# openshift/kubernetes-autoscaler

Hardware: NVIDIA H100
Metric: pod x node predicate evals/sec (higher is better)
Workload: dtype int64

## Files before the change

### kubernetes-autoscaler_b200/csrc/engine.h

```cpp
#pragma once
#include <cuda_runtime.h>

#include <climits>
#include <cstdint>
#include <string>
#include <vector>

#include "../../include/caengine.h"
#include "dyn.cuh"
#include "tables.cuh"

namespace cae {

constexpr int FEAS_MAX_W = 4;
constexpr int FEAS_LUT_MAX_ROWS = 1024;
constexpr int FEAS_TW = 16;

void set_error(const std::string& msg);

struct alignas(16) GroupRec {
  int32_t n, spec, sc, dc;
  uint32_t flags;
  int32_t pad[2];
  int32_t kcap;
  unsigned long long pconf, pbit;
  int64_t req[CAE_MAX_RES];
  float rinv[CAE_MAX_RES];
};
static_assert(sizeof(GroupRec) == 144, "GroupRec is fetched as nine 16-byte chunks");
enum : uint32_t { GREC_HAS_PORTS = 1u, GREC_FEEDS = 2u, GREC_HOST_SPREAD = 4u };

struct GroupRecSrc {
  int has_dyn, n_act;
  int act_dim[CAE_MAX_RES];
  const int32_t *spec_sc, *spec_dc, *pc_of;
  const unsigned long long* port_conf;
};
__device__ __forceinline__ GroupRec build_group_rec(const DevObjects& o, const GroupRecSrc& s, int spec, int n, bool feeds) {
  GroupRec r{};
  r.n = n;
  r.kcap = INT_MAX;
  if (n <= 0) return r;
  r.spec = spec;
  r.sc = s.spec_sc[spec];
  r.dc = s.has_dyn ? s.spec_dc[spec] : 0;
  const int plist = o.ps_port_list[spec];
  const bool has_ports = o.port_off[plist + 1] > o.port_off[plist];
  r.pconf = has_ports ? s.port_conf[plist] : 0ull;
  r.pbit = has_ports ? (1ull << s.pc_of[plist]) : 0ull;
  r.flags = (has_ports ? GREC_HAS_PORTS : 0u) | (feeds ? GREC_FEEDS : 0u) | (o.ps_hostname_spread[spec] ? GREC_HOST_SPREAD : 0u);
  for (int a = 0; a < s.n_act; ++a) {
    r.req[a] = o.ps_req[(size_t)spec * R + s.act_dim[a]];
    r.rinv[a] = r.req[a] > 0 ? __frcp_rn(__ll2float_rn(r.req[a])) : 0.f;
    if (r.req[a] >> 32) r.kcap = min(r.kcap, (int)(LLONG_MAX / r.req[a]));
  }
  return r;
}
constexpr int ORDER_NOT_ON_FRESH = 1 << 30;

#define CAE_CUDA(expr)                                                                        \
  do {                                                                                        \
    cudaError_t _e = (expr);                                                                  \
    if (_e != cudaSuccess) {                                                                  \
      cae::set_error(std::string(#expr) + ": " + cudaGetErrorString(_e));                     \
      return -1;                                                                              \
    }                                                                                         \
  } while (0)

#define CAE_KERNEL_OK()                                                                       \
  do {                                                                                        \
    cudaError_t _e = cudaGetLastError();                                                      \
    if (_e != cudaSuccess) {                                                                  \
      cae::set_error(std::string(__func__) + ": " + cudaGetErrorString(_e));                  \
      return -1;                                                                              \
    }                                                                                         \
  } while (0)

struct Arena {
  struct Chunk { void* dev = nullptr; void* host = nullptr; size_t size = 0, used = 0, flushed = 0; };
  std::vector<Chunk> chunks;
  size_t cur = 0;
  size_t min_chunk = (size_t)32 << 20;
  bool mirrored = false;
  int alloc(void** dev, void** stage, size_t bytes);
  int flush(cudaStream_t st, int64_t* bytes);
  void reset();
  void release();
};

struct Engine {
  cae_config cfg{};
  cudaStream_t stream = nullptr;
  cudaEvent_t ev0 = nullptr, ev1 = nullptr, ev2 = nullptr, ev3 = nullptr;
  Arena up;
  Arena pup;
  Arena scratch;
  Engine() { up.mirrored = true; pup.mirrored = true; }
  DynTables dyn;
  const uint8_t* d_spec_used = nullptr;
  const int32_t* d_dc_ngroups = nullptr;
  int64_t* d_c_free = nullptr;
  int32_t* d_c_slots = nullptr;
  cae_stats stats{};
  bool loaded = false;

  int N = 0, T = 0, E = 0, P = 0, U = 0;
  int A = 0;
  int act_dim[CAE_MAX_RES] = {0};
  int SC = 0, DC = 0;
  int Tw = 0;
  int Twp = 0;
  int p_begin = 0, p_end = 0;
  int t_begin = 0, t_end = 0;
  int Pl = 0, Plw = 0;
  bool has_dynamic = false;

  DevObjects dobj{};
  StaticClass* d_sclass = nullptr;
  uint8_t* d_pre_code = nullptr;
  uint32_t* d_pre_ok = nullptr;
  int32_t* d_spec_sc = nullptr;
  int32_t* d_spec_dc = nullptr;
  uint8_t* d_post_code = nullptr;
  uint32_t* d_post_ok = nullptr;
  int W = 0;
  uint32_t* d_spec_w = nullptr;
  uint32_t* d_pod_w = nullptr;
  uint16_t* d_pod_row = nullptr;
  int feas_B = 0;
  uint32_t feas_fstart = 0;
  uint8_t feas_sword[32] = {0}, feas_sshift[32] = {0};
  uint32_t* d_tslice = nullptr;
  int lut_rows = 0;
  int lut_base[CAE_MAX_RES] = {0};
  uint8_t lut_word[CAE_MAX_RES] = {0}, lut_shift[CAE_MAX_RES] = {0};
  uint32_t lut_mask[CAE_MAX_RES] = {0};
  uint32_t* d_rlut = nullptr;
  long long* d_tmpl_cost = nullptr;
  int32_t* d_perm = nullptr;
  bool force_bitslice = false;
  int32_t* d_pod_sc = nullptr;
  int32_t* d_pod_dc = nullptr;
  int64_t* d_tmpl_free = nullptr;
  int64_t* d_tmpl_free_all = nullptr;
  int32_t* d_tmpl_slots = nullptr;
  uint32_t* d_fit_bits = nullptr;
  uint8_t* d_reasons = nullptr;
  int32_t* d_fit_count = nullptr;
  int32_t* d_fit_acc = nullptr;
  int32_t* d_chunk_done = nullptr;
  uint8_t* d_group_reason = nullptr;
  bool group_reason_valid = false;
  int32_t* d_counts2 = nullptr;
  int32_t* d_sched = nullptr;
  int32_t* d_order = nullptr;
  int32_t* d_order_n = nullptr;
  GroupRec* d_grec = nullptr;
  double* d_waste = nullptr;
  int32_t* d_max_nodes = nullptr;
  int32_t* d_last_index_buf = nullptr;
  const int32_t* d_last_index_in = nullptr;
  int32_t* d_last_index_out = nullptr;
  int32_t* d_pc_of = nullptr;
  unsigned long long* d_port_conf = nullptr;
  int pack_cap = 1 << 30;
  struct DevBuf {
    void* p = nullptr;
    size_t cap = 0;
    DevBuf() = default;
    DevBuf(const DevBuf&) = delete;
    DevBuf& operator=(const DevBuf&) = delete;
    ~DevBuf() { if (p) cudaFree(p); }
  };
  struct PinnedBuf {
    void* p = nullptr;
    size_t cap = 0;
    cudaEvent_t ev = nullptr;
    PinnedBuf() = default;
    PinnedBuf(const PinnedBuf&) = delete;
    PinnedBuf& operator=(const PinnedBuf&) = delete;
    ~PinnedBuf() { if (p) cudaFreeHost(p); if (ev) cudaEventDestroy(ev); }
  };
  struct Slab { DevBuf buf; size_t sig = 0, zeroed = 0; };
  Slab pack_slab, fm_slab;
  DevBuf fm_blob;
  DevBuf rm_state;
  PinnedBuf rm_stage;
  std::vector<int32_t> rm_owner, rm_seen;
  DevBuf x_rows;
  DevBuf x_price;
  static constexpr int PEER_MAX = 8, PEER_CAP = 1 << 16;
  int32_t* d_xbuf = nullptr;
  int peer_world = 0;
  int32_t* peer_base[PEER_MAX] = {nullptr};
  int64_t peer_step = 0;
  int32_t* d_work_counter = nullptr;
  const int32_t *h_group_off = nullptr, *h_pend_spec = nullptr;
  std::vector<int32_t> h_group_spec;
  bool groups_homogeneous = true;
  std::vector<uint8_t> h_spec_pending;
  int cap_P = 0, cap_E = 0, cap_Pl = 0;
  PinnedBuf pending_stage;
  std::vector<int64_t> h_spec_req;
  int num_podspecs = 0;
  struct NodeHost {
    int32_t num_values = 0, num_labelsets = 0, num_taint_lists = 0, taint_entries = 0;
    std::vector<int32_t> ls_off, ls_key, ls_val;
    std::vector<int32_t> pod_cnt;
    int64_t pod_total = 0;
    std::vector<uint8_t> spec_used;
    std::vector<uint8_t> spec_anti;
    std::vector<int32_t> key_val;
    std::vector<int32_t> tkey_val;
    std::vector<int32_t> q_k;
    std::vector<int32_t> dom_scratch;
    std::vector<int32_t> tmpl_ls;
  } nh;
  struct PodHost {
    int32_t hostname_key = -1, num_res = 0;
    int32_t num_namespaces = 0, num_reqs = 0, req_vals = 0, num_selectors = 0, num_naff = 0, num_naff_terms = 0, fields = 0;
    int32_t num_tol_lists = 0, tol_entries = 0, num_aterms = 0, aterm_ns = 0;
    std::vector<int32_t> ps_namespace, ps_labelset, ps_tol_list, ps_naff, ps_node_name, ps_port_list, ps_pts_list, ps_aff_list,
        ps_anti_list;
    std::vector<int32_t> port_off, pts_off, pts_key, aff_off, aterm_key;
  } ph;
  DevBuf pd_tab[49];
  PinnedBuf pd_stage;
  DevBuf pd_blob;
  DevBuf pd_used;
  DevBuf nd_tab[9];
  DevBuf nd_off[2], nd_spec[2];
  DevBuf nd_cnt, nd_didx, nd_cub, nd_blob;
  PinnedBuf nd_stage;
  DevBuf ch_nodes[2];
  DevBuf ch_pre;
  DevBuf ch_dyn;
  DevBuf sim_dev;
  PinnedBuf sim_stage;
  int sm_count = 132;
  int smem_optin = 227 * 1024;
  size_t hbm_bytes = (size_t)80 << 30;
};

int devbuf_reserve(Engine* e, Engine::DevBuf& b, size_t bytes);
int pinned_reserve(Engine* e, Engine::PinnedBuf& b, size_t bytes);

int launch_class_matrix(Engine* e);
int launch_class_matrix_cols(Engine* e, const int32_t* d_cols, int ncols);
int launch_dynamic_recount(Engine* e, const int32_t* d_cols, int ncols);
struct NodeDeltaDev {
  int nd, na;
  const int32_t *row, *name;
  const int32_t *labelset, *taint_list, *allowed, *cslots, *pod_off, *pod_spec;
  const uint8_t* unsched;
  const int64_t *alloc, *cfree;
};
int launch_node_rows(Engine* e, const NodeDeltaDev& d, int64_t total);
int launch_node_churn(Engine* e, const NodeDeltaDev& d, const int32_t* src, int N_new, int64_t total);
int launch_pre_ok_bits(Engine* e);
int launch_post_bits(Engine* e);
int launch_dynamic_tables(Engine* e, const uint8_t* d_spec_used, const int32_t* d_dc_ngroups);
int launch_expand_pods(Engine* e);
int launch_port_conflicts(Engine* e, int num_port_lists);
int launch_feasibility(Engine* e, bool want_reasons);
int launch_group_feasibility(Engine* e);
int launch_order(Engine* e);
int launch_group_records(Engine* e);
GroupRecSrc group_rec_src(const Engine* e);
int launch_binpack(Engine* e);
struct FilterLaunch {
  int runs, n_pods, last_index, break_on_failure, nctrl;
  const int32_t *run_off, *pods, *hint, *cls, *class_ctrl;
  const uint8_t* node_ok;
  int32_t *assigned, *out, *ctrl_cnt;
  uint8_t *class_mark, *ctrl_over;
};
int launch_filter(Engine* e, const FilterLaunch& f);
struct RemovalLaunch {
  int ncand, persist, ncls, nctrl, log_cap, last_index, n_move;
  const int32_t *cand, *move_off, *move_pod, *hint, *cls, *class_ctrl;
  const uint8_t* dest_ok;
  int32_t *result, *log, *out;
};
struct RemovalState {
  int ncand, persist, log_cap, li_in, ncls, nctrl;
  const int32_t *cand, *move_off, *move_pod;
  const uint8_t* dest_ok;
  int32_t *result, *log, *out;
  int64_t* cfree;
  int32_t* cslots;
  unsigned long long* cports;
  uint8_t *live, *live_w;
  int32_t* rank;
  int32_t *ccnt, *cpres, *ctot;
  int32_t *wcnt, *wpres, *wtot;
  int32_t* stat;
  int32_t* hint;
  int32_t *head, *tail, *next;
  int32_t* run_off;
  GroupRecSrc grs;
};
int launch_removals(Engine* e, const RemovalLaunch& r);
struct RankArgs {
  int A, N, T, Tw, Twp, W, lut_rows, feas_B, Bpad;
  int act[CAE_MAX_RES], f_word[CAE_MAX_RES], f_shift[CAE_MAX_RES], f_bits[CAE_MAX_RES], lut_base[CAE_MAX_RES];
  uint32_t lut_mask[CAE_MAX_RES];
  int rv_off[CAE_MAX_RES + 1];
  uint8_t sword[32], sshift[32];
};
int launch_rank_tables(Engine* e, const RankArgs& a, const int64_t* d_rvals, uint32_t* d_tmpl_w);
int pd_resident_specs(Engine* e, int S, uint8_t* h_used, int32_t* h_labelset);
int launch_price(Engine* e, const cae_price_inputs& in_dev, const int32_t* d_node_count, const int32_t* d_sched, const int32_t* d_order,
                 double* d_score);
int launch_waste(Engine* e, const int32_t* d_node_count, const int32_t* d_sched, double* d_waste);
constexpr int SIM_KMAX = 2 * CAE_MAX_RES + 3;
struct SimLaunch {
  double ratio[3];
  const int32_t *res_sig, *lab_sig, *free_dims;
  int32_t* flags;
  const int64_t* cap;
  int32_t* status;
  unsigned long long* sum;
  int32_t* count;
  uint32_t* bits;
  double* x;
  uint32_t* sched;
};
int launch_similar(Engine* e, const SimLaunch& s);

}
```

### kubernetes-autoscaler_b200/csrc/feas.cu

```cuda
#include <algorithm>
#include <climits>

#include "engine.h"

namespace cae {

struct LutLayout {
  int A, rows;
  int base[CAE_MAX_RES];
  uint32_t mask[CAE_MAX_RES];
  uint8_t word[CAE_MAX_RES], shift[CAE_MAX_RES];
};

static LutLayout lut_layout(const Engine* e) {
  LutLayout lay{};
  lay.A = e->A;
  lay.rows = e->lut_rows;
  for (int d = 0; d < e->A; ++d) {
    lay.base[d] = e->lut_base[d]; lay.mask[d] = e->lut_mask[d]; lay.word[d] = e->lut_word[d]; lay.shift[d] = e->lut_shift[d];
  }
  return lay;
}

__global__ void expand_pods_kernel(const int32_t* __restrict__ pend_spec, int p_begin, int Pl, int W, LutLayout lay,
                                   const uint32_t* __restrict__ spec_w, const int32_t* __restrict__ spec_sc,
                                   const int32_t* __restrict__ spec_dc, uint32_t* __restrict__ pod_w,
                                   uint16_t* __restrict__ pod_row, int32_t* __restrict__ pod_sc, int32_t* __restrict__ pod_dc) {
  int p = blockIdx.x * blockDim.x + threadIdx.x;
  if (p >= Pl) return;
  int spec = pend_spec[p_begin + p];
  for (int w = 0; w < W; ++w) pod_w[(size_t)w * Pl + p] = spec_w[(size_t)spec * FEAS_MAX_W + w];
  for (int d = 0; d < lay.A; ++d) {
    const int row = lay.base[d] + (int)((spec_w[(size_t)spec * FEAS_MAX_W + lay.word[d]] >> lay.shift[d]) & lay.mask[d]);
    pod_row[(size_t)d * Pl + p] = (uint16_t)min(row, 0xFFFF);
  }
  pod_sc[p] = spec_sc[spec];
  pod_dc[p] = spec_dc[spec];
}

int launch_expand_pods(Engine* e) {
  if (e->Pl == 0) return 0;
  expand_pods_kernel<<<(e->Pl + 255) / 256, 256, 0, e->stream>>>(e->dobj.pend_spec, e->p_begin, e->Pl, e->W, lut_layout(e), e->d_spec_w,
                                                                   e->d_spec_sc, e->d_spec_dc, e->d_pod_w, e->d_pod_row, e->d_pod_sc, e->d_pod_dc);
  e->stats.kernel_launches++;
  CAE_KERNEL_OK();
  return 0;
}

constexpr int K1_TW = FEAS_TW;
constexpr int K1_TCHUNK = K1_TW * 32;
constexpr int K1_LPITCH = K1_TW + 1;

struct PeerPush {
  int world, rank;
  int tag;
  int2* data[8];
  const int2* self;
  int32_t* done_ctr;
  int32_t* status;
};

struct K1Args {
  int Pl, Plw, T, Tw, Twp, N, U, W;
  int G, gq, gr;
  const uint32_t* pod_w;
  const uint16_t* pod_row;
  const int32_t *pod_sc, *pod_dc;
  const uint32_t *tslice, *rlut;
  const int32_t* tmpl_slots;
  const uint32_t *pre_ok, *post_ok;
  const uint8_t *pre_code, *post_code;
  uint32_t* fit_bits;
  int32_t *fit_count, *fit_acc, *chunk_done;
  uint8_t* reasons;
};

__device__ __forceinline__ int k1_ld_acquire_sys(const int32_t* p) {
  int v;
  asm volatile("ld.acquire.sys.global.s32 %0, [%1];" : "=r"(v) : "l"(p) : "memory");
  return v;
}
__device__ __forceinline__ void k1_red_release_sys(int32_t* p, int v) {
  asm volatile("red.release.sys.global.add.s32 [%0], %1;" ::"l"(p), "r"(v) : "memory");
}
__device__ __forceinline__ void k1_st_volatile_v2(int2* p, int x, int y) {
  asm volatile("st.volatile.global.v2.s32 [%0], {%1, %2};" ::"l"(p), "r"(x), "r"(y) : "memory");
}
__device__ __forceinline__ int2 k1_ld_volatile_v2(const int2* p) {
  int2 v;
  asm volatile("ld.volatile.global.v2.s32 {%0, %1}, [%2];" : "=r"(v.x), "=r"(v.y) : "l"(p) : "memory");
  return v;
}
__device__ __forceinline__ unsigned long long k1_globaltimer() {
  unsigned long long t;
  asm volatile("mov.u64 %0, %%globaltimer;" : "=l"(t));
  return t;
}

#ifdef CAE_K1_PROF
constexpr int K1_PROF_MAX_BLOCKS = 8192, K1_PROF_STAMPS = 5;
__device__ unsigned long long k1_prof[1 + K1_PROF_STAMPS * K1_PROF_MAX_BLOCKS];
#define K1_STAMP(i)                                                                                 \
  do {                                                                                              \
    const int b_ = blockIdx.y * gridDim.x + blockIdx.x;                                             \
    if (threadIdx.x == 0 && b_ < K1_PROF_MAX_BLOCKS) k1_prof[1 + K1_PROF_STAMPS * b_ + (i)] = k1_globaltimer(); \
  } while (0)
__global__ void k1_prof_mark_kernel() { k1_prof[0] = k1_globaltimer(); }
#else
#define K1_STAMP(i) do {} while (0)
#endif

__device__ __forceinline__ void k1_finish(const K1Args& a, const PeerPush& pp, const int32_t* s_cnt, int t0, int tid, int nthreads) {
  __shared__ int s_flag;
  for (int i = tid; i < K1_TCHUNK; i += nthreads) {
    const int c = s_cnt[i];
    if (c && t0 + i < a.T) atomicAdd(&a.fit_acc[t0 + i], c);
  }
  __syncthreads();
  if (tid == 0) {
    __threadfence();
    s_flag = atomicAdd(&a.chunk_done[blockIdx.y], 1) == (int)gridDim.x - 1;
  }
  __syncthreads();
  if (!s_flag) return;
  __threadfence();
  for (int i = tid; i < K1_TCHUNK; i += nthreads) {
    const int t = t0 + i;
    if (t < a.T) {
      a.fit_count[t] = __ldcg(&a.fit_acc[t]);
      a.fit_acc[t] = 0;
    }
  }
  if (tid == 0) a.chunk_done[blockIdx.y] = 0;
  if (!pp.world) return;
  __syncthreads();
  if (tid == 0) {
    __threadfence();
    s_flag = atomicAdd(pp.done_ctr, 1) == (int)gridDim.y - 1;
  }
  __syncthreads();
  if (!s_flag) return;
  __threadfence();
  const int tag = pp.tag;
#pragma unroll
  for (int r = 0; r < Engine::PEER_MAX; ++r) {
    if (r < pp.world) {
      int2* dst = pp.data[r] + (size_t)pp.rank * Engine::PEER_CAP;
      for (int t = tid; t < a.T; t += nthreads) k1_st_volatile_v2(dst + t, __ldcg(&a.fit_count[t]), tag);
    }
  }
  const int2* mine = pp.self;
  const unsigned long long t0ns = k1_globaltimer();
  int ok = 1;
  for (int t = tid; t < a.T && ok; t += nthreads) {
    int2 x[Engine::PEER_MAX];
    unsigned pending = 0;
#pragma unroll
    for (int r = 0; r < Engine::PEER_MAX; ++r)
      if (r < pp.world) x[r] = k1_ld_volatile_v2(mine + (size_t)r * Engine::PEER_CAP + t);
#pragma unroll
    for (int r = 0; r < Engine::PEER_MAX; ++r)
      if (r < pp.world && x[r].y != tag) pending |= 1u << r;
    for (int spins = 0; pending; ) {
#pragma unroll
      for (int r = 0; r < Engine::PEER_MAX; ++r)
        if ((pending >> r) & 1u) {
          x[r] = k1_ld_volatile_v2(mine + (size_t)r * Engine::PEER_CAP + t);
          if (x[r].y == tag) pending &= ~(1u << r);
        }
      if (pending && (++spins & 1023) == 0 && k1_globaltimer() - t0ns > 2000000000ull) { ok = 0; break; }
    }
    int v = 0;
#pragma unroll
    for (int r = 0; r < Engine::PEER_MAX; ++r)
      if (r < pp.world) v += x[r].x;
    if (ok) a.fit_count[t] = v;
  }
  if (!ok) atomicExch(pp.status, 1);
  if (tid == 0) *pp.done_ctr = 0;
}

struct TransposeConsts { uint32_t sel16, sel8, amt[3], keep[3]; };

__device__ __forceinline__ uint32_t opaque(uint32_t v) {
  uint32_t r;
  asm volatile("mov.b32 %0, %1;" : "=r"(r) : "r"(v));
  return r;
}

__device__ __forceinline__ TransposeConsts transpose_consts(int lane) {
  TransposeConsts c;
  c.sel16 = opaque((lane & 16) ? 0x3276u : 0x5410u);
  c.sel8 = opaque((lane & 8) ? 0x3715u : 0x6240u);
#pragma unroll
  for (int i = 0; i < 3; ++i) {
    const int s = 4 >> i;
    const uint32_t lowmask = s == 4 ? 0x0F0F0F0Fu : s == 2 ? 0x33333333u : 0x55555555u;
    c.amt[i] = opaque((lane & s) ? (uint32_t)s : (uint32_t)(32 - s));
    c.keep[i] = opaque((lane & s) ? ~lowmask : lowmask);
  }
  return c;
}

__device__ __forceinline__ uint32_t bitselect(uint32_t x, uint32_t y, uint32_t keep) {
  uint32_t r;
  asm("lop3.b32 %0, %1, %2, %3, 0xE4;" : "=r"(r) : "r"(x), "r"(y), "r"(keep));
  return r;
}

__device__ __forceinline__ void warp_transpose32x2(uint32_t& a, uint32_t& b, const TransposeConsts& c) {
  uint32_t ya = __shfl_xor_sync(0xffffffffu, a, 16), yb = __shfl_xor_sync(0xffffffffu, b, 16);
  a = __byte_perm(a, ya, c.sel16);
  b = __byte_perm(b, yb, c.sel16);
  ya = __shfl_xor_sync(0xffffffffu, a, 8);
  yb = __shfl_xor_sync(0xffffffffu, b, 8);
  a = __byte_perm(a, ya, c.sel8);
  b = __byte_perm(b, yb, c.sel8);
#pragma unroll
  for (int i = 0; i < 3; ++i) {
    ya = __shfl_xor_sync(0xffffffffu, __funnelshift_l(a, a, c.amt[i]), 4 >> i);
    yb = __shfl_xor_sync(0xffffffffu, __funnelshift_l(b, b, c.amt[i]), 4 >> i);
    a = bitselect(a, ya, c.keep[i]);
    b = bitselect(b, yb, c.keep[i]);
  }
}

__device__ __forceinline__ uint32_t warp_transpose32(uint32_t x, int lane) {
#pragma unroll
  for (int s = 16; s >= 1; s >>= 1) {
    const uint32_t lowmask = s == 16 ? 0x0000FFFFu : s == 8 ? 0x00FF00FFu : s == 4 ? 0x0F0F0F0Fu : s == 2 ? 0x33333333u : 0x55555555u;
    const uint32_t y = __shfl_xor_sync(0xffffffffu, x, s);
    x = (lane & s) ? ((x & ~lowmask) | ((y & ~lowmask) >> s)) : ((x & lowmask) | ((y & lowmask) << s));
  }
  return x;
}

template <int A, bool REASONS>
constexpr int k1_lut_warps_per_sm() { return REASONS ? 16 : (A == 0 || A > 5) ? 32 : 48; }

template <int A, bool REASONS, int NW>
__global__ void __launch_bounds__(NW * 32, k1_lut_warps_per_sm<A, REASONS>() / NW)
feasibility_lut_kernel(K1Args a, int rows, PeerPush pp) {
  extern __shared__ uint32_t k1_smem[];
  constexpr int NT = NW * 32;
  constexpr int PAD = K1_TCHUNK + 32 / NW;
  uint32_t* s_lut = k1_smem;
  uint32_t* s_out = s_lut + (size_t)max(rows, 1) * K1_LPITCH;
  int32_t* s_cnt = reinterpret_cast<int32_t*>(s_out + NW * PAD);
  const int tid = threadIdx.x, lane = tid & 31, warp = tid >> 5;
  const int tw0 = blockIdx.y * K1_TW;
  const int t0 = tw0 * 32;
  const int pwb = (int)blockIdx.x * a.gq + min((int)blockIdx.x, a.gr);
  const int npw = a.gq + ((int)blockIdx.x < a.gr ? 1 : 0);
  const int p = (pwb + warp) * 32 + lane;
  const bool valid = warp < npw && p < a.Pl;
  K1_STAMP(0);

#pragma unroll 1
  for (int i = tid; i < rows * K1_TW; i += NT) {
    const int row = i / K1_TW, w = i % K1_TW;
    s_lut[row * K1_LPITCH + w] = a.rlut[(size_t)row * a.Twp + tw0 + w];
  }
  for (int i = tid; i < K1_TCHUNK; i += NT) s_cnt[i] = 0;

  int off[A > 0 ? A : 1];
#pragma unroll
  for (int d = 0; d < A; ++d) off[d] = valid ? (int)a.pod_row[(size_t)d * a.Pl + p] * K1_LPITCH : 0;
  const int sc = valid ? a.pod_sc[p] : 0;
  const int dc = valid ? a.pod_dc[p] : 0;
  uint32_t cls[K1_TW];
  {
    const uint4* pre = reinterpret_cast<const uint4*>(a.pre_ok + (size_t)sc * a.Twp + tw0);
    const uint4* post = reinterpret_cast<const uint4*>(a.post_ok + (size_t)dc * a.Twp + tw0);
#pragma unroll
    for (int q = 0; q < K1_TW / 4; ++q) {
      uint4 u = make_uint4(0, 0, 0, 0);
      if (valid) {
        const uint4 x = __ldg(pre + q), y = __ldg(post + q);
        u = make_uint4(x.x & y.x, x.y & y.y, x.z & y.z, x.w & y.w);
      }
      cls[4 * q + 0] = u.x; cls[4 * q + 1] = u.y; cls[4 * q + 2] = u.z; cls[4 * q + 3] = u.w;
    }
  }
  const TransposeConsts tc = transpose_consts(lane);
  __syncthreads();
  K1_STAMP(1);

#pragma unroll
  for (int tw = 0; tw < K1_TW; tw += 2) {
    uint32_t fit0 = 0xffffffffu, fit1 = 0xffffffffu;
#pragma unroll
    for (int d = 0; d < A; ++d) {
      fit0 &= s_lut[off[d] + tw];
      fit1 &= s_lut[off[d] + tw + 1];
    }
    if (REASONS) {
#pragma unroll
      for (int h = 0; h < 2; ++h) {
        const int wglob = tw0 + tw + h;
        const uint32_t fit = h ? fit1 : fit0;
        if (valid && wglob < a.Tw) {
          for (int j = 0; j < 32; ++j) {
            const int t = wglob * 32 + j;
            if (t >= a.T) break;
            uint8_t rs = a.pre_code[(size_t)sc * a.U + a.N + t] & 0x0F;
            if (rs == 0) rs = (!((fit >> j) & 1u) || a.tmpl_slots[t] < 1) ? CAE_R_FIT : a.post_code[(size_t)dc * a.T + t];
            a.reasons[(size_t)t * a.Pl + p] = rs;
          }
        }
      }
    }
    uint32_t c0 = fit0 & cls[tw], c1 = fit1 & cls[tw + 1];
    warp_transpose32x2(c0, c1, tc);
    s_out[warp * PAD + tw * 32 + lane] = c0;
    s_out[warp * PAD + (tw + 1) * 32 + lane] = c1;
    atomicAdd(&s_cnt[tw * 32 + lane], __popc(c0));
    atomicAdd(&s_cnt[(tw + 1) * 32 + lane], __popc(c1));
  }
  __syncthreads();
  K1_STAMP(2);
  if (a.fit_bits) {
    const int wv = tid % NW;
    if (wv < npw) {
      uint32_t* dst = a.fit_bits + (size_t)(t0 + tid / NW) * a.Plw + pwb + wv;
      const uint32_t* src = s_out + wv * PAD + tid / NW;
      const size_t stride = (size_t)32 * a.Plw;
      const int kmax = min(K1_TCHUNK / 32, (a.T - t0 - tid / NW + 31) / 32);
#pragma unroll 4
      for (int k = 0; k < kmax; ++k, dst += stride, src += 32) *dst = *src;
    }
  }
  K1_STAMP(3);
  k1_finish(a, pp, s_cnt, t0, tid, NT);
  K1_STAMP(4);
}

constexpr int K1_THREADS = 256;
constexpr int K1_WARPS = K1_THREADS / 32;
constexpr int K1_PAD = K1_TCHUNK + 4;

struct FeasLayout {
  uint32_t fstart;
  int nb;
  uint8_t sword[32], sshift[32];
};

template <int B, bool REASONS>
__global__ void __launch_bounds__(K1_THREADS)
feasibility_kernel(K1Args a, FeasLayout lay, PeerPush pp) {
  __shared__ uint32_t s_sl[B > 0 ? B : 1][K1_TW];
  __shared__ uint32_t s_out[K1_WARPS][K1_PAD];
  __shared__ int32_t s_cnt[K1_TCHUNK];
  const int tid = threadIdx.x, lane = tid & 31, warp = tid >> 5;
  const int p = blockIdx.x * K1_THREADS + tid;
  const int tw0 = blockIdx.y * K1_TW;
  const int t0 = tw0 * 32;

  for (int i = tid; i < B * K1_TW; i += K1_THREADS) {
    const int b = i / K1_TW, w = i % K1_TW;
    s_sl[b][w] = (tw0 + w < a.Tw) ? a.tslice[(size_t)b * a.Tw + tw0 + w] : 0u;
  }
  for (int i = tid; i < K1_TCHUNK; i += K1_THREADS) s_cnt[i] = 0;
  const bool valid = p < a.Pl;
  uint32_t r[B > 0 ? B : 1];
  {
    uint32_t pw[FEAS_MAX_W];
#pragma unroll
    for (int w = 0; w < FEAS_MAX_W; ++w) pw[w] = (valid && w < a.W) ? a.pod_w[(size_t)w * a.Pl + p] : 0u;
#pragma unroll
    for (int b = 0; b < B; ++b) {
      const uint32_t word = lay.sword[b] == 0 ? pw[0] : lay.sword[b] == 1 ? pw[1] : lay.sword[b] == 2 ? pw[2] : pw[3];
      r[b] = b < lay.nb ? 0u - ((word >> lay.sshift[b]) & 1u) : 0u;
    }
  }
  const int sc = valid ? a.pod_sc[p] : 0;
  const int dc = valid ? a.pod_dc[p] : 0;
  __syncthreads();

#pragma unroll 1
  for (int tw = 0; tw < K1_TW; ++tw) {
    const int wglob = tw0 + tw;
    uint32_t row = 0;
    if (wglob < a.Tw) {
      uint32_t gt = 0, eq = 0;
#pragma unroll
      for (int b = 0; b < B; ++b) {
        const uint32_t f = s_sl[b][tw];
        if ((lay.fstart >> b) & 1u) eq = 0xffffffffu;
        gt |= eq & r[b] & ~f;
        eq &= ~(r[b] ^ f);
      }
      row = valid ? (~gt & a.pre_ok[(size_t)sc * a.Twp + wglob] & a.post_ok[(size_t)dc * a.Twp + wglob]) : 0u;
      if (REASONS) {
        if (valid) {
          for (int j = 0; j < 32; ++j) {
            const int t = wglob * 32 + j;
            if (t >= a.T) break;
            uint8_t rs = a.pre_code[(size_t)sc * a.U + a.N + t] & 0x0F;
            if (rs == 0) rs = (((gt >> j) & 1u) || a.tmpl_slots[t] < 1) ? CAE_R_FIT : a.post_code[(size_t)dc * a.T + t];
            a.reasons[(size_t)t * a.Pl + p] = rs;
          }
        }
      }
    }
    const uint32_t col = warp_transpose32(row, lane);
    s_out[warp][tw * 32 + lane] = col;
    if (col) atomicAdd(&s_cnt[tw * 32 + lane], __popc(col));
  }
  __syncthreads();
  const int pw0 = blockIdx.x * K1_WARPS;
  for (int i = tid; i < K1_TCHUNK * K1_WARPS; i += K1_THREADS) {
    const int tl = i / K1_WARPS, wv = i % K1_WARPS;
    const int t = t0 + tl;
    if (t < a.T && pw0 + wv < a.Plw && a.fit_bits) a.fit_bits[(size_t)t * a.Plw + pw0 + wv] = s_out[wv][tl];
  }
  k1_finish(a, pp, s_cnt, t0, tid, K1_THREADS);
}

static PeerPush peer_push_args(Engine* e) {
  PeerPush pp{};
  if (e->peer_world > 1 && e->T <= Engine::PEER_CAP) {
    const int par = (int)(e->peer_step & 1);
    const size_t blk = (size_t)Engine::PEER_MAX * Engine::PEER_CAP;
    pp.world = e->peer_world;
    pp.rank = e->cfg.rank;
    e->peer_step += 1;
    pp.tag = (int)(e->peer_step & 0x7fffffff);
    if (pp.tag == 0) pp.tag = 1;
    for (int r = 0; r < e->peer_world; ++r) pp.data[r] = reinterpret_cast<int2*>(e->peer_base[r]) + par * blk;
    pp.self = pp.data[pp.rank];
    pp.done_ctr = e->d_xbuf + 4 * blk + 8;
    pp.status = e->d_xbuf + 4 * blk + 9;
  }
  return pp;
}

static K1Args k1_args(Engine* e) {
  K1Args a{};
  a.Pl = e->Pl; a.Plw = e->Plw; a.T = e->T; a.Tw = e->Tw; a.Twp = e->Twp; a.N = e->N; a.U = e->U; a.W = e->W;
  a.G = 1;
  a.pod_w = e->d_pod_w; a.pod_row = e->d_pod_row; a.pod_sc = e->d_pod_sc; a.pod_dc = e->d_pod_dc;
  a.tslice = e->d_tslice; a.rlut = e->d_rlut; a.tmpl_slots = e->d_tmpl_slots;
  a.pre_ok = e->d_pre_ok; a.post_ok = e->d_post_ok; a.pre_code = e->d_pre_code; a.post_code = e->d_post_code;
  a.fit_bits = e->d_fit_bits; a.fit_count = e->d_fit_count; a.fit_acc = e->d_fit_acc; a.chunk_done = e->d_chunk_done;
  a.reasons = e->d_reasons;
  return a;
}

template <int B>
static void launch_feas_b(Engine* e, bool want_reasons, K1Args a, const PeerPush& pp) {
  dim3 grid((e->Pl + K1_THREADS - 1) / K1_THREADS, e->Twp / K1_TW);
  FeasLayout lay;
  lay.fstart = e->feas_fstart;
  lay.nb = e->feas_B;
  for (int b = 0; b < 32; ++b) { lay.sword[b] = e->feas_sword[b]; lay.sshift[b] = e->feas_sshift[b]; }
  if (want_reasons) feasibility_kernel<B, true><<<grid, K1_THREADS, 0, e->stream>>>(a, lay, pp);
  else feasibility_kernel<B, false><<<grid, K1_THREADS, 0, e->stream>>>(a, lay, pp);
}

template <int A, bool REASONS, int NW>
static int launch_feas_lut_arw(Engine* e, K1Args a, const PeerPush& pp) {
  const int chunks = e->Twp / K1_TW;
  const int slots = e->sm_count * (k1_lut_warps_per_sm<A, REASONS>() / NW);
  const int g_min = (e->Plw + NW - 1) / NW;
  a.G = std::max(g_min, std::min(e->Plw, std::max(1, slots / chunks)));
  a.gq = e->Plw / a.G;
  a.gr = e->Plw % a.G;
  dim3 grid(a.G, chunks);
  const size_t smem = sizeof(uint32_t) * ((size_t)std::max(e->lut_rows, 1) * K1_LPITCH + NW * (K1_TCHUNK + 32 / NW) + K1_TCHUNK);
  auto kern = feasibility_lut_kernel<A, REASONS, NW>;
  if (smem > 48 * 1024) CAE_CUDA(cudaFuncSetAttribute(kern, cudaFuncAttributeMaxDynamicSharedMemorySize, (int)smem));
  kern<<<grid, NW * 32, smem, e->stream>>>(a, e->lut_rows, pp);
  return 0;
}

template <int A>
static int launch_feas_lut_a(Engine* e, bool want_reasons, const K1Args& a, const PeerPush& pp) {
  return want_reasons ? launch_feas_lut_arw<A, true, 16>(e, a, pp) : launch_feas_lut_arw<A, false, 16>(e, a, pp);
}

constexpr int K1_LUT_MAX_ROWS = FEAS_LUT_MAX_ROWS;

int launch_feasibility(Engine* e, bool want_reasons) {
  if (e->Tw == 0) return 0;
  if (e->Pl == 0) {
    CAE_CUDA(cudaMemsetAsync(e->d_fit_count, 0, sizeof(int32_t) * e->T, e->stream));
    return 0;
  }
  if (e->peer_world > 1 && e->T > Engine::PEER_CAP) {
    set_error("fused histogram exchange: more templates than the exchange buffer holds (use the NCCL all-reduce of cae_device_buffer(0))");
    return 1;
  }
#ifdef CAE_K1_PROF
  {
    void* prof = nullptr;
    CAE_CUDA(cudaGetSymbolAddress(&prof, k1_prof));
    CAE_CUDA(cudaMemsetAsync(prof, 0, sizeof(k1_prof), e->stream));
    k1_prof_mark_kernel<<<1, 1, 0, e->stream>>>();
  }
#endif
  const PeerPush pp = peer_push_args(e);
  const K1Args a = k1_args(e);
  if (!e->force_bitslice && e->lut_rows <= K1_LUT_MAX_ROWS) {
    int rc = 0;
    switch (e->A) {
      case 0: rc = launch_feas_lut_a<0>(e, want_reasons, a, pp); break;
      case 1: rc = launch_feas_lut_a<1>(e, want_reasons, a, pp); break;
      case 2: rc = launch_feas_lut_a<2>(e, want_reasons, a, pp); break;
      case 3: rc = launch_feas_lut_a<3>(e, want_reasons, a, pp); break;
      case 4: rc = launch_feas_lut_a<4>(e, want_reasons, a, pp); break;
      case 5: rc = launch_feas_lut_a<5>(e, want_reasons, a, pp); break;
      case 6: rc = launch_feas_lut_a<6>(e, want_reasons, a, pp); break;
      case 7: rc = launch_feas_lut_a<7>(e, want_reasons, a, pp); break;
      default: rc = launch_feas_lut_a<8>(e, want_reasons, a, pp); break;
    }
    if (rc) return rc;
  } else {
    const int Bp = e->feas_B == 0 ? 0 : (e->feas_B + 3) / 4 * 4;
    switch (Bp) {
      case 0: launch_feas_b<0>(e, want_reasons, a, pp); break;
      case 4: launch_feas_b<4>(e, want_reasons, a, pp); break;
      case 8: launch_feas_b<8>(e, want_reasons, a, pp); break;
      case 12: launch_feas_b<12>(e, want_reasons, a, pp); break;
      case 16: launch_feas_b<16>(e, want_reasons, a, pp); break;
      case 20: launch_feas_b<20>(e, want_reasons, a, pp); break;
      case 24: launch_feas_b<24>(e, want_reasons, a, pp); break;
      case 28: launch_feas_b<28>(e, want_reasons, a, pp); break;
      default: launch_feas_b<32>(e, want_reasons, a, pp); break;
    }
  }
  e->stats.kernel_launches++;
  CAE_KERNEL_OK();
  return 0;
}

}

#ifdef CAE_K1_PROF
extern "C" int cae_k1_prof_read(unsigned long long* out, int n) {
  n = std::max(0, std::min(n, 1 + cae::K1_PROF_STAMPS * cae::K1_PROF_MAX_BLOCKS));
  if (cudaMemcpyFromSymbol(out, cae::k1_prof, sizeof(unsigned long long) * n) != cudaSuccess) return -1;
  return n;
}
#endif
```

Before: 5041 billion.

## Fuse per-template count reduction with arrival counter in 64-bit atomics

Each template's global accumulator becomes 64-bit, with the high bits counting arriving blocks and the low bits summing fit counts. When the whole grid fits in one wave and no peer push is active, the last-arriving block writes the final count directly, so the chunk-level done counter, fences and extra barrier pass are skipped. The arrival atomic is issued early so its latency overlaps with the fit_bits stores. The shared-memory per-template counters are also packed two per word, halving the shared atomics. This adds 64-bit global atomic traffic and a second code path chosen by the `elect` flag.

```diff
diff --git a/kubernetes-autoscaler_b200/csrc/engine.h b/kubernetes-autoscaler_b200/csrc/engine.h
--- a/kubernetes-autoscaler_b200/csrc/engine.h
+++ b/kubernetes-autoscaler_b200/csrc/engine.h
@@ -147,7 +147,7 @@
   uint32_t* d_fit_bits = nullptr;
   uint8_t* d_reasons = nullptr;
   int32_t* d_fit_count = nullptr;
-  int32_t* d_fit_acc = nullptr;
+  unsigned long long* d_fit_acc = nullptr;
   int32_t* d_chunk_done = nullptr;
   uint8_t* d_group_reason = nullptr;
   bool group_reason_valid = false;
diff --git a/kubernetes-autoscaler_b200/csrc/feas.cu b/kubernetes-autoscaler_b200/csrc/feas.cu
--- a/kubernetes-autoscaler_b200/csrc/feas.cu
+++ b/kubernetes-autoscaler_b200/csrc/feas.cu
@@ -71,7 +71,10 @@
   const uint32_t *pre_ok, *post_ok;
   const uint8_t *pre_code, *post_code;
   uint32_t* fit_bits;
-  int32_t *fit_count, *fit_acc, *chunk_done;
+  int32_t* fit_count;
+  unsigned long long* fit_acc;
+  int32_t* chunk_done;
+  int elect;
   uint8_t* reasons;
 };
 
@@ -110,28 +113,45 @@
 #define K1_STAMP(i) do {} while (0)
 #endif
 
-__device__ __forceinline__ void k1_finish(const K1Args& a, const PeerPush& pp, const int32_t* s_cnt, int t0, int tid, int nthreads) {
+constexpr unsigned long long K1_ARRIVAL = 1ull << 40;
+
+__device__ __forceinline__ unsigned long long k1_block_count(const uint32_t* s_cnt2, int i) {
+  return (s_cnt2[(i >> 6) * 32 + (i & 31)] >> (i & 32 ? 16 : 0)) & 0xFFFFu;
+}
+
+__device__ __forceinline__ unsigned long long k1_acc_arrive(const K1Args& a, int t, unsigned long long c) {
+  return atomicAdd(&a.fit_acc[t], K1_ARRIVAL | c);
+}
+
+__device__ __forceinline__ void k1_acc_done(const K1Args& a, int t, unsigned long long old, unsigned long long c) {
+  if (a.elect) {
+    if (c) atomicAdd(&a.fit_acc[t], c);
+  } else if (old / K1_ARRIVAL == gridDim.x - 1) {
+    a.fit_count[t] = (int32_t)(old % K1_ARRIVAL + c);
+    a.fit_acc[t] = 0;
+  }
+}
+
+__device__ __forceinline__ void k1_finish(const K1Args& a, const PeerPush& pp, int t0, int tid, int nthreads) {
   __shared__ int s_flag;
-  for (int i = tid; i < K1_TCHUNK; i += nthreads) {
-    const int c = s_cnt[i];
-    if (c && t0 + i < a.T) atomicAdd(&a.fit_acc[t0 + i], c);
-  }
-  __syncthreads();
-  if (tid == 0) {
+  if (a.elect) {
+    __syncthreads();
+    if (tid == 0) {
+      __threadfence();
+      s_flag = atomicAdd(&a.chunk_done[blockIdx.y], 1) == (int)gridDim.x - 1;
+    }
+    __syncthreads();
+    if (!s_flag) return;
     __threadfence();
-    s_flag = atomicAdd(&a.chunk_done[blockIdx.y], 1) == (int)gridDim.x - 1;
-  }
-  __syncthreads();
-  if (!s_flag) return;
-  __threadfence();
-  for (int i = tid; i < K1_TCHUNK; i += nthreads) {
-    const int t = t0 + i;
-    if (t < a.T) {
-      a.fit_count[t] = __ldcg(&a.fit_acc[t]);
-      a.fit_acc[t] = 0;
-    }
-  }
-  if (tid == 0) a.chunk_done[blockIdx.y] = 0;
+    for (int i = tid; i < K1_TCHUNK; i += nthreads) {
+      const int t = t0 + i;
+      if (t < a.T) {
+        a.fit_count[t] = (int32_t)__ldcg(&a.fit_acc[t]);
+        a.fit_acc[t] = 0;
+      }
+    }
+    if (tid == 0) a.chunk_done[blockIdx.y] = 0;
+  }
   if (!pp.world) return;
   __syncthreads();
   if (tid == 0) {
@@ -246,7 +266,7 @@
   constexpr int PAD = K1_TCHUNK + 32 / NW;
   uint32_t* s_lut = k1_smem;
   uint32_t* s_out = s_lut + (size_t)max(rows, 1) * K1_LPITCH;
-  int32_t* s_cnt = reinterpret_cast<int32_t*>(s_out + NW * PAD);
+  uint32_t* s_cnt2 = s_out + NW * PAD;
   const int tid = threadIdx.x, lane = tid & 31, warp = tid >> 5;
   const int tw0 = blockIdx.y * K1_TW;
   const int t0 = tw0 * 32;
@@ -261,7 +281,7 @@
     const int row = i / K1_TW, w = i % K1_TW;
     s_lut[row * K1_LPITCH + w] = a.rlut[(size_t)row * a.Twp + tw0 + w];
   }
-  for (int i = tid; i < K1_TCHUNK; i += NT) s_cnt[i] = 0;
+  for (int i = tid; i < K1_TCHUNK / 2; i += NT) s_cnt2[i] = 0;
 
   int off[A > 0 ? A : 1];
 #pragma unroll
@@ -314,11 +334,14 @@
     warp_transpose32x2(c0, c1, tc);
     s_out[warp * PAD + tw * 32 + lane] = c0;
     s_out[warp * PAD + (tw + 1) * 32 + lane] = c1;
-    atomicAdd(&s_cnt[tw * 32 + lane], __popc(c0));
-    atomicAdd(&s_cnt[(tw + 1) * 32 + lane], __popc(c1));
+    atomicAdd(&s_cnt2[tw * 16 + lane], __popc(c0) | __popc(c1) << 16);
   }
   __syncthreads();
   K1_STAMP(2);
+  static_assert(NT == K1_TCHUNK, "one template of the chunk per thread");
+  const bool own = t0 + tid < a.T;
+  const unsigned long long c = own ? k1_block_count(s_cnt2, tid) : 0;
+  const unsigned long long old = own && !a.elect ? k1_acc_arrive(a, t0 + tid, c) : 0;
   if (a.fit_bits) {
     const int wv = tid % NW;
     if (wv < npw) {
@@ -331,7 +354,8 @@
     }
   }
   K1_STAMP(3);
-  k1_finish(a, pp, s_cnt, t0, tid, NT);
+  if (own) k1_acc_done(a, t0 + tid, old, c);
+  k1_finish(a, pp, t0, tid, NT);
   K1_STAMP(4);
 }
 
@@ -414,7 +438,13 @@
     const int t = t0 + tl;
     if (t < a.T && pw0 + wv < a.Plw && a.fit_bits) a.fit_bits[(size_t)t * a.Plw + pw0 + wv] = s_out[wv][tl];
   }
-  k1_finish(a, pp, s_cnt, t0, tid, K1_THREADS);
+  for (int i = tid; i < K1_TCHUNK; i += K1_THREADS) {
+    if (t0 + i < a.T) {
+      const unsigned long long c = (unsigned)s_cnt[i];
+      k1_acc_done(a, t0 + i, a.elect ? 0 : k1_acc_arrive(a, t0 + i, c), c);
+    }
+  }
+  k1_finish(a, pp, t0, tid, K1_THREADS);
 }
 
 static PeerPush peer_push_args(Engine* e) {
@@ -450,6 +480,7 @@
 template <int B>
 static void launch_feas_b(Engine* e, bool want_reasons, K1Args a, const PeerPush& pp) {
   dim3 grid((e->Pl + K1_THREADS - 1) / K1_THREADS, e->Twp / K1_TW);
+  a.elect = grid.x * grid.y > (unsigned)e->sm_count || pp.world;
   FeasLayout lay;
   lay.fstart = e->feas_fstart;
   lay.nb = e->feas_B;
@@ -466,8 +497,9 @@
   a.G = std::max(g_min, std::min(e->Plw, std::max(1, slots / chunks)));
   a.gq = e->Plw / a.G;
   a.gr = e->Plw % a.G;
+  a.elect = a.G * chunks > slots || pp.world;
   dim3 grid(a.G, chunks);
-  const size_t smem = sizeof(uint32_t) * ((size_t)std::max(e->lut_rows, 1) * K1_LPITCH + NW * (K1_TCHUNK + 32 / NW) + K1_TCHUNK);
+  const size_t smem = sizeof(uint32_t) * ((size_t)std::max(e->lut_rows, 1) * K1_LPITCH + NW * (K1_TCHUNK + 32 / NW) + K1_TCHUNK / 2);
   auto kern = feasibility_lut_kernel<A, REASONS, NW>;
   if (smem > 48 * 1024) CAE_CUDA(cudaFuncSetAttribute(kern, cudaFuncAttributeMaxDynamicSharedMemorySize, (int)smem));
   kern<<<grid, NW * 32, smem, e->stream>>>(a, e->lut_rows, pp);
```

Result: faster. 5287 billion, median of 6 (+4.9%).
